# YonghaoHe/LFD-A-Light-and-Fast-Detector

Measured on NVIDIA H100. Metric: images/sec WIDERFACE-S inference 1280x720 batch=8 per GPU bf16, higher is better.
Workload: dtype bf16

## Files before the change

### lfd-a-light-and-fast-detector_b200/build.py

```python
import os
import subprocess
import sys

HERE = os.path.dirname(os.path.abspath(__file__))
CSRC = os.path.join(HERE, 'csrc')
OUT = os.environ.get('LFD_B200_OUT') or os.path.join(HERE, 'liblfd_b200.so')
SOURCES = ['api.cu', 'conv_umma.cu', 'conv_simt.cu', 'postprocess.cu', 'losses.cu', 'train.cu', 'wgrad_umma.cu', 'input.cu']
HEADERS = ['ptx.cuh', 'conv_common.cuh', 'kernels.cuh', 'train.cuh', os.path.join('..', '..', 'include', 'lfd_b200.h')]
NVCC = os.environ.get('NVCC', '/usr/local/cuda/bin/nvcc')
ARCH = ['-gencode', 'arch=compute_90a,code=sm_90a']
FLAGS = ARCH + ['-O3', '-lineinfo', '-std=c++17', '-Xcompiler', '-fPIC',
                '--expt-relaxed-constexpr'] + (['-DLFD_B200_TRACE'] if os.environ.get('LFD_B200_TRACE') else []) + \
        (['-DLFD_B200_TIMELINE'] if os.environ.get('LFD_B200_TIMELINE') else []) + os.environ.get('LFD_B200_EXTRA_FLAGS', '').split()


def _stale():
    if not os.path.exists(OUT):
        return True
    t = os.path.getmtime(OUT)
    deps = [os.path.join(CSRC, s) for s in SOURCES + HEADERS] + [os.path.abspath(__file__)]
    return any(os.path.getmtime(d) > t for d in deps)


_STACK_GUARDED = ('conv_umma_kernel', 'conv_umma_c48_kernel', 'stem4_kernel', 'soft_nms_kernel')
_WGMMA_GUARDED = ('conv_umma_kernel', 'conv_umma_c48_kernel', 'stem4_kernel')
_PTXAS_VERBOSE = ('conv_umma.cu', 'postprocess.cu')


def _check_stack_frames(ptxas_log, limit=64):
    import re
    name = None
    for line in ptxas_log.splitlines():
        m = re.search(r'Function properties for (\S+)', line)
        if m:
            name = m.group(1)
        m = re.search(r'(\d+) bytes stack frame', line)
        if m and name and any(k in name for k in _STACK_GUARDED) and int(m.group(1)) > limit:
            raise RuntimeError('%s has a %s-byte stack frame (limit %d): registers went to local memory' % (name, m.group(1), limit))
        m = re.search(r'\((C75\d\d)\).*wgmma\.mma_async instructions are serialized.*\'(\S+)\'', line)
        if m and any(k in m.group(2) for k in _WGMMA_GUARDED):
            raise RuntimeError('ptxas serialised the wgmma instructions of %s (%s):\n%s' % (m.group(2), m.group(1), line))


def build(force=False, verbose=False):
    if not force and not _stale():
        return OUT
    objs = []
    procs = []
# ... 22 lines not shown
```

### lfd-a-light-and-fast-detector_b200/csrc/conv_common.cuh

```cuda
#pragma once
#include <cuda.h>
#include <cuda_runtime.h>
#include <cuda_bf16.h>
#include <stdint.h>
#include <string.h>
#include "kernels.cuh"

namespace lfd {

enum { MODE_FLAT = 0, MODE_3X3S1 = 1, MODE_3X3S2 = 2, MODE_1X1S2 = 3, MODE_STEM = 4, MODE_STEM4 = 5 };

static constexpr int kMaxStages = 8;
static constexpr int kMaxDevices = 64;
static constexpr int kSmemBarOff = 0;
static constexpr int kSmemTableOff = 512;

struct ConvGeom {
    int N, H, W, Cin, Ho, Wo, Cout, ksize, stride;
    int tail_cout;
    int ds_cout;
    int stem;
    int stem4;
};

// ... 18 lines not shown
    unsigned long long* tl;
    long long* trace;
    int N, H, W, Cin, Ho, Wo, Cout;
    int relu, gn_groups, mode;
    int tiles_x, tiles_per_img, num_tiles;
    unsigned long long magic_tpi, magic_tx;
    int n_px;
    int Cc, stages, b_resident;
    int log2_cpc, log2_cpr;
    uint32_t lbo_a, sbo_a;
    uint32_t a_stage_bytes, b_slice_bytes, stage_bytes, w_total_bytes;
    uint32_t smem_table_off, smem_bias_off, smem_bias2_off, smem_staging_off;
    uint32_t smem_w_off, smem_ring_off;
    int input_format;
    InputTransform xf;
    int f16;
    const __nv_bfloat16* w_s2;
    const float* shift_s2;
    const __nv_bfloat16* w_s3;
    const float* shift_s3;
    int relu_s2, relu_s3, H1, W1;
    int in_words;
    const int* ext;
};

int umma_conv_configure(const ConvGeom& g, int num_sms, UmmaConvParams* out, size_t* smem_bytes, int* grid);
cudaError_t umma_conv_launch(const UmmaConvParams& p, size_t smem, int grid, cudaStream_t st);
int umma_conv_encode_maps(UmmaConvParams* p);

cudaError_t simt_conv_launch(const ConvGeom& g, int Cc, const __nv_bfloat16* in, __nv_bfloat16* out,
                             const __nv_bfloat16* res, const __nv_bfloat16* w, const float* shift,
                             double* stats, int gn_groups, int relu, int f16, cudaStream_t st);

}
```

### lfd-a-light-and-fast-detector_b200/csrc/conv_umma.cu

```cuda
#include <stdlib.h>

#include <type_traits>

#include "conv_common.cuh"
#include "ptx.cuh"

namespace lfd {

static constexpr int kProdThreads = 128;
static constexpr int kConsumerThreads = 256;
static constexpr int kConvThreads = kConsumerThreads + kProdThreads;

#define LFD_LAMBDA_INLINE __attribute__((always_inline))

#ifdef LFD_B200_TRACE
#define LFD_TRACE(role, idx, slot) \
    do { if (p.trace && blockIdx.x == 0 && (idx) < 32) p.trace[((role) * 32 + (idx)) * 4 + (slot)] = clock64(); } while (0)
#define LFD_TRACE_EPI(tr, idx, slot) \
    do { if ((tr) && blockIdx.x == 0 && (idx) < 16) (tr)[(idx) * 8 + (slot)] = clock64(); } while (0)
#else
#define LFD_TRACE(role, idx, slot) ((void)0)
#define LFD_TRACE_EPI(tr, idx, slot) ((void)0)
#endif

// ... 18 lines not shown
    if (MODE == MODE_FLAT) {
        g.tiles_x = 0; g.magic_tx = 0;
        g.tiles_per_img = (g.Ho * p.Wo + 127) / 128;
    } else {
        g.tiles_x = (g.Wo + 7) / 8;
        g.magic_tx = ((1ull << 40) + (uint64_t)g.tiles_x - 1) / (uint64_t)g.tiles_x;
        g.tiles_per_img = g.tiles_x * ((g.Ho + 15) / 16);
    }
    g.num_tiles = g.tiles_per_img * p.N;
    g.magic_tpi = ((1ull << 40) + (uint64_t)g.tiles_per_img - 1) / (uint64_t)g.tiles_per_img;
    return g;
}

struct PxEntry {
    uint32_t src_off;
    uint32_t dst_off;
};
struct PxDelta { int8_t dy, dx; };

static constexpr int kStemRows = 33, kStemCols = 18, kStemPix = kStemRows * kStemCols;
static constexpr int kStemRowBytes = kStemCols * 8;
static constexpr int kStemPerThread = (kStemPix + kProdThreads - 1) / kProdThreads;
static constexpr int kStemPatchBytes = ((kStemRows * kStemRowBytes + 127) / 128) * 128;

LFD_DEVINL float selp_f32(bool c, float a, float b) {
    float r;
    asm("{\n\t.reg .pred p;\n\tsetp.ne.u32 p, %3, 0;\n\tselp.f32 %0, %1, %2, p;\n\t}" : "=f"(r) : "f"(a), "f"(b), "r"((uint32_t)c));
    return r;
}

template <int NV, int N>
LFD_DEVINL void butterfly_step(float* val, int lane) {
    if constexpr (N > 1) {
        constexpr int off = 16 * N / NV;
        const bool upper = (lane & off) != 0;
#pragma unroll
        for (int i = 0; i < N / 2; ++i) {
            const float lo = val[i], hi = val[i + N / 2];
            const float send = selp_f32(upper, lo, hi);
            const float keep = selp_f32(upper, hi, lo);
            val[i] = keep + __shfl_xor_sync(0xffffffffu, send, off);
        }
        butterfly_step<NV, N / 2>(val, lane);
    }
}

// ... 27 lines not shown
    return 0;
}

LFD_DEVINL void wg_bar_sync(int wg) { asm volatile("bar.sync %0, 128;" ::"r"(1 + wg) : "memory"); }

template <int N, int K, bool F16>
LFD_DEVINL void tail_mma(float* acc2, const uint32_t* a2, uint64_t b2desc0) {
#pragma unroll
    for (int kk = 0; kk < K / 16; ++kk) wgmma_rs<N, F16>(acc2, a2 + 4 * kk, b2desc0 + (uint32_t)((kk * 2 * N * 16) >> 4), kk != 0);
}

struct EpiCtx {
    uint32_t stg;
    uint32_t stg_bytes;
    int nbuf;
    int r0, tq;
    int wtid;
    int wg, lane;
#ifdef LFD_B200_TRACE
    long long* tr;
#endif
};

template <int MODE, int NCMAX, bool F16>
LFD_DEVINL void store_tile(const EpiCtx& e, const float* acc, int nc, const float* bias, bool relu, bool res, double* stats,
                           const CUtensorMap* tmap, const CUtensorMap* tmres, int c0, int c1, int n, bool v0, bool v1,
                           uint64_t* res_bar, uint32_t& store_count, uint32_t& res_count) {
    const uint32_t buf = e.stg + (e.nbuf == 2 ? (store_count & 1) * e.stg_bytes : 0u);
#ifdef LFD_B200_TRACE
    const uint32_t tidx = store_count;
#endif
    ++store_count;
    const int row_bytes = nc >= 64 ? 128 : nc * 2;
    const int n_panels = nc >= 64 ? nc / 64 : 1;
    if (e.wtid == 0) {
        LFD_TRACE_EPI(e.tr, tidx, 0);
        if (e.nbuf == 2) bulk_wait_read<1>(); else bulk_wait_read<0>();
        LFD_TRACE_EPI(e.tr, tidx, 1);
        if (res) {
            mbar_arrive_expect_tx(res_bar, 64u * nc * 2u);
            for (int pn = 0; pn < n_panels; ++pn) {
                if (MODE == MODE_FLAT) tma_load_3d(buf + pn * 8192, tmres, pn * 64, c0, n, res_bar);
                else tma_load_4d(buf + pn * 8192, tmres, pn * 64, c0, c1, n, res_bar);
            }
        }
    }
    constexpr int JB = NCMAX / 8 < 8 ? NCMAX / 8 : 4;
    float2 bv[JB];
    auto load_shifts = [&](int j0) LFD_LAMBDA_INLINE {
#pragma unroll
        for (int i = 0; i < JB; ++i)
            if (j0 + i < nc / 8) bv[i] = *reinterpret_cast<const float2*>(bias + 8 * (j0 + i) + 2 * e.tq);
    };
    load_shifts(0);
    wg_bar_sync(e.wg);
    if (res) { mbar_wait(res_bar, res_count & 1); ++res_count; }
    float st[NCMAX == 128 ? 32 : 1];
    const bool stat = NCMAX == 128 && stats != nullptr;
#pragma unroll
    for (int j = 0; j < NCMAX / 8; ++j) {
        if (j < nc / 8) {
            if (j > 0 && j % JB == 0) load_shifts(j);
            const float b0 = bv[j % JB].x, b1 = bv[j % JB].y;
            float s1 = 0.f, s2 = 0.f;
#pragma unroll
            for (int h = 0; h < 2; ++h) {
                const int row = e.r0 + 8 * h;
                const uint32_t swz = NCMAX == 48 ? 0u : (row_bytes == 128 ? (row & 7) : (row_bytes == 64 ? ((row >> 1) & 3) : ((row >> 2) & 1)));
                const uint32_t addr = buf + (uint32_t)(j >> 3) * 8192u + (uint32_t)(row * row_bytes) + ((((uint32_t)j & 7u) ^ swz) << 4) + 4u * e.tq;
                float x0 = acc[4 * j + 2 * h] + b0, x1 = acc[4 * j + 2 * h + 1] + b1;
                if (res) {
                    uint32_t rv;
                    asm volatile("ld.shared.b32 %0, [%1];" : "=r"(rv) : "r"(addr) : "memory");
                    x0 += up_lo<F16>(rv); x1 += up_hi<F16>(rv);
                }
                const uint32_t o = relu ? pack2_relu<F16>(x0, x1) : pack2<F16>(x0, x1);
                asm volatile("st.shared.b32 [%0], %1;" ::"r"(addr), "r"(o) : "memory");
                if (stat && (h ? v1 : v0)) {
                    const float f0 = up_lo<F16>(o), f1 = up_hi<F16>(o);
                    s1 += f0 + f1;
                    s2 = fmaf(f0, f0, fmaf(f1, f1, s2));
                }
            }
            if (NCMAX == 128) { st[j] = s1; st[16 + j] = s2; }
        }
    }
    fence_proxy_async_smem();
    wg_bar_sync(e.wg);
    if (e.wtid == 0) {
        for (int pn = 0; pn < n_panels; ++pn) {
            if (MODE == MODE_FLAT) tma_store_3d(tmap, buf + pn * 8192, pn * 64, c0, n);
            else tma_store_4d(tmap, buf + pn * 8192, pn * 64, c0, c1, n);
        }
        bulk_commit();
        LFD_TRACE_EPI(e.tr, tidx, 2);
    }
    if (NCMAX == 128 && stat) stats_flush<128>(st, e.lane, stats);
}

template <int MODE, int COUT, bool F16, bool EXT, bool DS>
LFD_DEVINL void conv_umma_body(const UmmaConvParams& p) {
    static_assert(!DS || MODE == MODE_3X3S2, "the fused shortcut belongs to a 3x3/s2 conv");
    constexpr int kProd = kProdThreads;
    constexpr int kThreads = kConvThreads;
    constexpr int TAPS = (MODE == MODE_3X3S1 || MODE == MODE_3X3S2) ? 9 : (MODE == MODE_STEM ? 3 : 1);
    extern __shared__ __align__(1024) uint8_t smem[];
    uint64_t* full = reinterpret_cast<uint64_t*>(smem + kSmemBarOff);
    uint64_t* empty = full + kMaxStages;
    uint64_t* wbar = empty + kMaxStages;
    uint64_t* res_bar = wbar + 1;
    PxEntry* table = reinterpret_cast<PxEntry*>(smem + p.smem_table_off);
    PxDelta* delta = reinterpret_cast<PxDelta*>(smem + p.smem_table_off + (size_t)p.n_px * sizeof(PxEntry));
    float* bias = reinterpret_cast<float*>(smem + p.smem_bias_off);
    float* bias2 = reinterpret_cast<float*>(smem + p.smem_bias2_off);
    uint8_t* staging = smem + p.smem_staging_off;
    uint8_t* wres = smem + p.smem_w_off;
    uint8_t* ring = smem + p.smem_ring_off;

    pdl_launch_dependents();
    LFD_TL_BEGIN(p.tl);
    const int tid = threadIdx.x;
    const int warp = tid >> 5;
    const int lane = tid & 31;
    const int SA = p.stages;
    const int cpc = p.Cc >> 3;
// ... 68 lines not shown
        e.tq = lane & 3;
        e.wtid = tid & 127;
        e.wg = wg;
        e.lane = lane;
#ifdef LFD_B200_TRACE
        e.tr = p.trace && e.wtid == 0 ? p.trace + (3 * 32 + wg) * 4 : nullptr;
#endif
        if (e.wtid == 0 && (e.stg & 1023u)) __trap();

        const uint32_t lbo_b = COUT * 16;
        const uint64_t adesc0 = wgmma_desc(0, p.lbo_a, p.sbo_a);
        const uint64_t bdesc0 = wgmma_desc(0, lbo_b, 128);
        const uint32_t a_k16 = (2 * p.lbo_a) >> 4;
        const uint32_t b_k16 = (2 * lbo_b) >> 4;
        const uint32_t b_tap = (cpc * lbo_b) >> 4;
        const uint32_t a_wg = (8u * p.sbo_a * wg) >> 4;
        const int nk16 = p.Cc >> 4;
        const uint64_t b2desc0 = wgmma_desc(smem_u32(smem + p.smem_w2_off), cn2 * 16, 128);
        const int flat_valid = lg.Ho * p.Wo;

        float acc[COUT / 2];
        float acc3[DS ? COUT / 2 : 1];
        uint32_t it = 0, store_count = 0, res_count = 0;
        for (int tile = blockIdx.x, lt = 0; tile < lg.num_tiles; tile += gridDim.x, ++lt) {
            for (int cc = 0; cc < n_cc; ++cc, ++it) {
                const uint32_t s = it % SA, ph = (it / SA) & 1;
                if (cc == 0 && e.wtid == 0) LFD_TRACE(1 + wg, lt, 0);
                mbar_wait(&full[s], ph);
                if (e.wtid == 0) LFD_TRACE(1 + wg, lt, 1);
                fence_proxy_async_smem();
                const uint32_t a_base = smem_u32(ring) + s * p.stage_bytes;
                const uint32_t b_base = p.b_resident ? smem_u32(wres) + cc * p.b_slice_bytes : a_base + p.a_stage_bytes;
                const uint64_t ad = adesc0 + ((a_base >> 4) + a_wg), bd = bdesc0 + (b_base >> 4);
                wgmma_fence_regs<COUT / 2>(acc);
                wgmma_fence();
                for (int k16 = 0; k16 < nk16; ++k16) {
                    const uint64_t adk = ad + (uint32_t)(k16 * a_k16), bdk = bd + (uint32_t)(k16 * b_k16);
#pragma unroll
                    for (int tap = 0; tap < TAPS; ++tap)
                        wgmma_ss<COUT, F16>(acc, adk + (uint32_t)tap_view<MODE>(tap), bdk + (uint32_t)(tap * b_tap), (cc | k16 | tap) != 0);
                }
                if constexpr (DS) {
                    wgmma_fence_regs<COUT / 2>(acc3);
                    for (int k16 = 0; k16 < nk16; ++k16)
                        wgmma_ss<COUT, F16>(acc3, ad + (uint32_t)(k16 * a_k16) + (uint32_t)tap_view<MODE>(4),
                                            b2desc0 + (uint32_t)(((cc * cpc + 2 * k16) * COUT * 16) >> 4), (cc | k16) != 0);
// ... 170 lines not shown
                const int ty = fast_div(t, lg.magic_tx);
                int oy0 = ty * 16, ox0 = (t - ty * lg.tiles_x) * 8;
                iy0 = (MODE == MODE_3X3S1) ? oy0 : 2 * oy0;
                ix0 = (MODE == MODE_3X3S1) ? ox0 : 2 * ox0;
            }
            const __nv_bfloat16* img = p.in + (size_t)n * HW * p.Cin + ch * 8;
            constexpr int kDyMin = (MODE == MODE_1X1S2) ? 0 : -1, kDxMin = kDyMin;
            constexpr int kDyMax = (MODE == MODE_3X3S1) ? 16 : ((MODE == MODE_3X3S2) ? 31 : 30);
            constexpr int kDxMax = (MODE == MODE_3X3S1) ? 8 : ((MODE == MODE_3X3S2) ? 15 : 14);
            const bool interior = MODE == MODE_FLAT ? (ix0 + 128 <= HW)
                                                    : (iy0 + kDyMin >= 0 && ix0 + kDxMin >= 0 && iy0 + kDyMax < lg.H && ix0 + kDxMax < lg.W);
            const __nv_bfloat16* org = img + (ptrdiff_t)(MODE == MODE_FLAT ? ix0 : (iy0 + kDyMin) * p.W + ix0 + kDxMin) * p.Cin;
            for (int cc = 0; cc < n_cc; ++cc, ++it) {
                const uint32_t s = it % SA, ph = (it / SA) & 1;
                if (ptid == 0) LFD_TRACE(0, it, 0);
                mbar_wait(&empty[s], ph ^ 1);
                if (ptid == 0) LFD_TRACE(0, it, 1);
                const uint32_t a_base = smem_u32(ring) + s * p.stage_bytes;
                if (!p.b_resident && ptid == 0) {
                    mbar_arrive_expect_tx(&full[s], p.b_slice_bytes);
                    bulk_g2s(a_base + p.a_stage_bytes, reinterpret_cast<const uint8_t*>(p.w) + (size_t)cc * p.b_slice_bytes,
                             p.b_slice_bytes, &full[s]);
                }
                const __nv_bfloat16* src_cc = img + cc * p.Cc;
                const uint32_t dst_cc = a_base + ch_dst;
                if (MODE == MODE_FLAT) {
                    if (interior) {
                        const __nv_bfloat16* src = org + cc * p.Cc + (size_t)px0 * p.Cin;
                        const size_t sstep = (size_t)pstep * p.Cin;
                        uint32_t dst = dst_cc + px0 * 16;
#pragma unroll 4
                        for (int pxi = px0; pxi < 128; pxi += pstep, src += sstep, dst += pstep * 16) cp_async16_full(dst, src);
                    } else {
#pragma unroll 4
                        for (int pxi = px0; pxi < 128; pxi += pstep) {
                            const int q = ix0 + pxi;
                            const bool ok = q < HW;
                            cp_async16(dst_cc + pxi * 16, src_cc + (ok ? q : 0) * p.Cin, ok);
                        }
                    }
                } else if (interior) {
                    const uint8_t* src = reinterpret_cast<const uint8_t*>(org + cc * p.Cc);
                    const PxEntry* tp = table + px0;
#pragma unroll 4
                    for (int k = 0; k < my_cnt; ++k, tp += pstep) {
                        const uint2 pe = *reinterpret_cast<const uint2*>(tp);
// ... 7 lines not shown
                        const bool ok = ((unsigned)y < (unsigned)lg.H) && ((unsigned)x < (unsigned)lg.W);
                        cp_async16(dst_cc + table[pxi].dst_off, src_cc + (ok ? (y * p.W + x) : 0) * p.Cin, ok);
                    }
                }
                cp_async_mbar_arrive(&full[s]);
                if (ptid == 0) LFD_TRACE(0, it, 2);
            }
        }
        cp_async_wait_all();
        }
    }
    LFD_TL_END(p.tl);
}

template <int MODE, int COUT, bool F16, bool EXT, bool DS>
__global__ void __launch_bounds__(kConvThreads, 1) conv_umma_kernel(const __grid_constant__ UmmaConvParams p) {
    static_assert(COUT != 48, "48-channel outputs run in conv_umma_c48_kernel");
    conv_umma_body<MODE, COUT, F16, EXT, DS>(p);
}

template <int MODE, bool F16, bool EXT, bool DS>
__global__ void __launch_bounds__(kConvThreads, 1) conv_umma_c48_kernel(const __grid_constant__ UmmaConvParams p) {
    conv_umma_body<MODE, 48, F16, EXT, DS>(p);
}

static constexpr int kS4Rows = 67, kS4Cols = 36, kS4Pix = kS4Rows * kS4Cols;
static constexpr int kS4RowBytes = kS4Cols * 8;
static constexpr int kS4PatchBytes = kS4Pix * 8;
static constexpr int kS4PerThread = (kS4Pix + kProdThreads - 1) / kProdThreads;
static constexpr int kS4Batch = 5;
static constexpr int kS4Groups = kS4Rows * 10;
static constexpr int kS4GroupsPerThread = (kS4Groups + kProdThreads - 1) / kProdThreads;
static constexpr int kS4GroupBatch = 3;
static constexpr int kS4PatchOverrun = 768;
LFD_DEVINL constexpr int s4_slot(int a, int b) {
    return ((a & 1) ? ((b & 1) ? 0 : 147) : ((b & 1) ? 291 : 446)) + (a >> 1) * 9 + (b >> 1);
}
static constexpr int kS4Lbo = 599 * 16;
static constexpr int kS4Bar = 0;
static constexpr int kS4Shift = 256;
static constexpr int kS4Staging = 2048;
static constexpr int kS4W0 = kS4Staging + 2 * 8192;
static constexpr int kS4W1 = kS4W0 + 6144;
static constexpr int kS4W2 = kS4W1 + 8192;
static constexpr int kS4W3 = kS4W2 + 73728;
static constexpr int kS4Planes = kS4W3 + 8192;
// ... 324 lines not shown
#pragma unroll
                    for (int j = 0; j < kS4Batch; ++j) {
                        const int q = ptid + (j0 + j) * kProdThreads;
                        if (q >= kS4Pix) break;
                        float f[3];
#pragma unroll
                        for (int k = 0; k < 3; ++k) {
                            f[k] = u8 ? p.xf.apply(k, raw[j][k]) : __uint_as_float(raw[j][k]);
                            if (!ok[j]) f[k] = 0.f;
                        }
                        const uint32_t lo = pack2<F16>(sw ? f[2] : f[0], f[1]), hi = pack2<F16>(sw ? f[0] : f[2], 0.f);
                        asm volatile("st.shared.v2.b32 [%0], {%1, %2};" ::"r"(dst0 + q * 8), "r"(lo), "r"(hi) : "memory");
                    }
                }
            }
            fence_proxy_async_smem();
            mbar_arrive(&full[s]);
            if (ptid == 0) LFD_TRACE(0, lt, 2);
        }
    }
    LFD_TL_END(p.tl);
}

static int configure_with(const ConvGeom& g, int num_sms, int nbuf, UmmaConvParams* out, size_t* smem_bytes, int* grid) {
    UmmaConvParams p;
    memset(&p, 0, sizeof(p));
    p.stg_nbuf = nbuf;
    int mode;
    if (g.stem) {
        if (g.ksize != 3 || g.stride != 2 || g.Cin != 16) return -1;
        mode = MODE_STEM;
    } else if (g.ksize == 1 && g.stride == 1) mode = MODE_FLAT;
    else if (g.ksize == 3 && g.stride == 1) mode = MODE_3X3S1;
    else if (g.ksize == 3 && g.stride == 2) mode = MODE_3X3S2;
    else if (g.ksize == 1 && g.stride == 2) mode = MODE_1X1S2;
    else return -1;
    if (g.Cin % 16 || (g.Cout != 16 && g.Cout != 32 && g.Cout != 48 && g.Cout != 64 && g.Cout != 128)) return -1;
    if ((mode == MODE_3X3S1 || mode == MODE_3X3S2) && g.Cout < 32) return -1;
    p.mode = mode;
    p.N = g.N; p.H = g.H; p.W = g.W; p.Cin = g.Cin; p.Ho = g.Ho; p.Wo = g.Wo; p.Cout = g.Cout;
    const int taps = g.stem ? 3 : g.ksize * g.ksize;
    int px_slots;
    if (mode == MODE_FLAT) {
        p.tiles_x = 0; p.tiles_per_img = (g.Ho * g.Wo + 127) / 128;
        p.n_px = 128; px_slots = 128; p.sbo_a = 128;
    } else {
        p.tiles_x = (g.Wo + 7) / 8;
        p.tiles_per_img = p.tiles_x * ((g.Ho + 15) / 16);
        if (mode == MODE_3X3S1) { p.n_px = 180; px_slots = 180; p.sbo_a = 160; }
        else if (mode == MODE_3X3S2) { p.n_px = 561; px_slots = 594; p.sbo_a = 144; }
        else { p.n_px = 128; px_slots = 128; p.sbo_a = 128; }
    }
    const int plane_slots = px_slots | 1;
    p.lbo_a = plane_slots * 16;
    if (mode == MODE_STEM) { p.lbo_a = 16; p.sbo_a = 2 * kStemRowBytes; }
    p.num_tiles = p.tiles_per_img * g.N;
    if (p.num_tiles >= (1 << 24) || p.tiles_per_img >= (1 << 16)) return -5;
    p.magic_tpi = ((1ull << 40) + p.tiles_per_img - 1) / p.tiles_per_img;
    p.magic_tx = p.tiles_x ? ((1ull << 40) + p.tiles_x - 1) / p.tiles_x : 0;
    const int Cf = g.tail_cout > 0 ? g.tail_cout : g.Cout;
    if (g.ds_cout && (mode != MODE_3X3S2 || g.tail_cout || g.ds_cout != g.Cout)) return -6;
    if (g.tail_cout && (g.tail_cout % 16 || g.tail_cout > 128 || g.tail_cout < 16)) return -4;
    if (g.tail_cout && (g.tail_cout == 48) != (g.Cout == 48)) return -4;
    const size_t staging = (size_t)nbuf * 128 * Cf * 2;
    size_t hoff = kSmemTableOff;
    p.smem_table_off = (uint32_t)hoff;
    if (mode != MODE_FLAT && mode != MODE_STEM) hoff += ((size_t)p.n_px * 10 + 127) & ~(size_t)127;
    p.smem_bias_off = (uint32_t)hoff; hoff += ((size_t)g.Cout * 4 + 15) & ~(size_t)15;
    p.smem_bias2_off = (uint32_t)hoff; hoff += ((size_t)(g.tail_cout + g.ds_cout) * 4 + 15) & ~(size_t)15;
    p.smem_staging_off = (uint32_t)((hoff + 1023) & ~(size_t)1023);
    const size_t fixed = p.smem_staging_off + staging;
    const size_t w2_bytes = g.tail_cout ? ((size_t)g.Cout * g.tail_cout * 2 + 127) & ~(size_t)127
                                        : (g.ds_cout ? ((size_t)g.Cin * g.ds_cout * 2 + 127) & ~(size_t)127 : 0);
    const size_t post = w2_bytes;
    const size_t budget = 224 * 1024 - post;
    const size_t w_total = (size_t)taps * g.Cin * g.Cout * 2;
// ... 114 lines not shown
    const cuuint32_t inner = p.Cf < 64 ? p.Cf : 64;
    const CUtensorMapSwizzle swz = inner * 2 >= 128 ? CU_TENSOR_MAP_SWIZZLE_128B
                                 : (inner * 2 == 96 ? CU_TENSOR_MAP_SWIZZLE_NONE
                                                    : (inner * 2 == 64 ? CU_TENSOR_MAP_SWIZZLE_64B : CU_TENSOR_MAP_SWIZZLE_32B));
    cuuint64_t dims[4], strides[3];
    cuuint32_t box[4], estr[4] = {1, 1, 1, 1};
    cuuint32_t rank;
    if (p.mode == MODE_FLAT) {
        rank = 3;
        dims[0] = Cf; dims[1] = HoWo; dims[2] = p.N;
        strides[0] = Cf * 2; strides[1] = HoWo * Cf * 2;
        box[0] = inner; box[1] = 64; box[2] = 1;
    } else {
        rank = 4;
        dims[0] = Cf; dims[1] = p.Wo; dims[2] = p.Ho; dims[3] = p.N;
        strides[0] = Cf * 2; strides[1] = (cuuint64_t)p.Wo * Cf * 2; strides[2] = HoWo * Cf * 2;
        box[0] = inner; box[1] = 8; box[2] = 8; box[3] = 1;
    }
    CUresult r = fn(tm, CU_TENSOR_MAP_DATA_TYPE_BFLOAT16, rank, const_cast<void*>(ptr), dims, strides, box, estr, CU_TENSOR_MAP_INTERLEAVE_NONE, swz,
                    CU_TENSOR_MAP_L2_PROMOTION_L2_128B, CU_TENSOR_MAP_FLOAT_OOB_FILL_NONE);
    return r == CUDA_SUCCESS ? 0 : -2;
}

int umma_conv_encode_maps(UmmaConvParams* p) {
    if (encode_one(*p, p->out, &p->tm_out)) return -1;
    if (p->res && encode_one(*p, p->res, &p->tm_res)) return -1;
    if (p->Cout3 && encode_one(*p, p->out3, &p->tm_out3)) return -1;
    return 0;
}

static cudaError_t launch_persistent(void (*kernel)(UmmaConvParams), bool* configured, int max_smem, const UmmaConvParams& p, size_t smem,
                                     int grid, cudaStream_t st) {
    int dev = 0;
    if (cudaGetDevice(&dev) != cudaSuccess || dev < 0 || dev >= kMaxDevices) return cudaErrorInvalidDevice;
    if (!configured[dev]) {
        cudaError_t e = cudaFuncSetAttribute(kernel, cudaFuncAttributeMaxDynamicSharedMemorySize, max_smem);
        if (e != cudaSuccess) return e;
        configured[dev] = true;
    }
    cudaLaunchConfig_t cfg;
    memset(&cfg, 0, sizeof(cfg));
    cfg.gridDim = dim3(grid);
    cfg.blockDim = dim3(kConvThreads);
    cfg.dynamicSmemBytes = smem;
    cfg.stream = st;
    cudaLaunchAttribute attr[1];
    attr[0].id = cudaLaunchAttributeProgrammaticStreamSerialization;
    attr[0].val.programmaticStreamSerializationAllowed = 1;
    cfg.attrs = attr;
    cfg.numAttrs = 1;
// ... 5 lines not shown
    static bool configured[kMaxDevices] = {};
    if constexpr (COUT == 48) return launch_persistent(conv_umma_c48_kernel<MODE, F16, EXT, DS>, configured, 224 * 1024, p, smem, grid, st);
    else return launch_persistent(conv_umma_kernel<MODE, COUT, F16, EXT, DS>, configured, 224 * 1024, p, smem, grid, st);
}

template <int MODE, int COUT, bool F16, bool EXT>
static cudaError_t launch_mode_ds(const UmmaConvParams& p, size_t smem, int grid, cudaStream_t st) {
    if constexpr (MODE == MODE_3X3S2)
        if (p.Cout3) return launch_mode_t<MODE, COUT, F16, EXT, true>(p, smem, grid, st);
    return launch_mode_t<MODE, COUT, F16, EXT, false>(p, smem, grid, st);
}

template <bool F16, bool EXT>
static cudaError_t launch_stem4_t(const UmmaConvParams& p, size_t smem, int grid, cudaStream_t st) {
    static bool configured[kMaxDevices] = {};
    return launch_persistent(stem4_kernel<F16, EXT>, configured, kS4Smem, p, smem, grid, st);
}

template <bool F16>
static cudaError_t launch_stem4(const UmmaConvParams& p, size_t smem, int grid, cudaStream_t st) {
    return p.ext ? launch_stem4_t<F16, true>(p, smem, grid, st) : launch_stem4_t<F16, false>(p, smem, grid, st);
}

template <int MODE, int COUT, bool F16>
static cudaError_t launch_mode_e(const UmmaConvParams& p, size_t smem, int grid, cudaStream_t st) {
    return p.ext ? launch_mode_ds<MODE, COUT, F16, true>(p, smem, grid, st) : launch_mode_ds<MODE, COUT, F16, false>(p, smem, grid, st);
}

template <int MODE, int COUT>
static cudaError_t launch_mode(const UmmaConvParams& p, size_t smem, int grid, cudaStream_t st) {
    return p.f16 ? launch_mode_e<MODE, COUT, true>(p, smem, grid, st) : launch_mode_e<MODE, COUT, false>(p, smem, grid, st);
}

template <int MODE>
static cudaError_t launch_cout(const UmmaConvParams& p, size_t smem, int grid, cudaStream_t st) {
    switch (p.Cout) {
        case 16: if constexpr (MODE != MODE_3X3S1 && MODE != MODE_3X3S2) return launch_mode<MODE, 16>(p, smem, grid, st); break;
        case 32: return launch_mode<MODE, 32>(p, smem, grid, st);
        case 48: return launch_mode<MODE, 48>(p, smem, grid, st);
        case 64: return launch_mode<MODE, 64>(p, smem, grid, st);
        case 128: if constexpr (MODE != MODE_STEM) return launch_mode<MODE, 128>(p, smem, grid, st); break;
    }
    return cudaErrorInvalidValue;
}

cudaError_t umma_conv_launch(const UmmaConvParams& p, size_t smem, int grid, cudaStream_t st) {
    switch (p.mode) {
        case MODE_FLAT: return launch_cout<MODE_FLAT>(p, smem, grid, st);
// ... 11 lines not shown
```

### lfd-a-light-and-fast-detector_b200/csrc/ptx.cuh

```cuda
#pragma once
#include <cuda_runtime.h>
#include <cuda_bf16.h>
#include <cuda_fp16.h>
#include <stdint.h>

namespace lfd {

#define LFD_DEVINL __device__ __forceinline__

#ifndef LFD_SPIN_LIMIT
#define LFD_SPIN_LIMIT (1u << 27)
#endif

LFD_DEVINL uint32_t smem_u32(const void* p) { return (uint32_t)__cvta_generic_to_shared(p); }

LFD_DEVINL void mbar_init(uint64_t* bar, uint32_t count) {
    asm volatile("mbarrier.init.shared::cta.b64 [%0], %1;" ::"r"(smem_u32(bar)), "r"(count));
}
LFD_DEVINL void fence_mbar_init() { asm volatile("fence.mbarrier_init.release.cluster;" ::: "memory"); }
LFD_DEVINL void mbar_arrive(uint64_t* bar) {
    asm volatile("mbarrier.arrive.shared::cta.b64 _, [%0];" ::"r"(smem_u32(bar)) : "memory");
}
LFD_DEVINL void mbar_arrive_expect_tx(uint64_t* bar, uint32_t bytes) {
    asm volatile("mbarrier.arrive.expect_tx.shared::cta.b64 _, [%0], %1;" ::"r"(smem_u32(bar)), "r"(bytes) : "memory");
// ... 57 lines not shown
    return pred != 0;
}

LFD_DEVINL void tma_store_3d(const void* tmap, uint32_t src_smem, int c0, int c1, int c2) {
    asm volatile("cp.async.bulk.tensor.3d.global.shared::cta.bulk_group [%0, {%1, %2, %3}], [%4];" ::"l"(tmap), "r"(c0), "r"(c1),
                 "r"(c2), "r"(src_smem)
                 : "memory");
}
LFD_DEVINL void tma_store_4d(const void* tmap, uint32_t src_smem, int c0, int c1, int c2, int c3) {
    asm volatile("cp.async.bulk.tensor.4d.global.shared::cta.bulk_group [%0, {%1, %2, %3, %4}], [%5];" ::"l"(tmap), "r"(c0),
                 "r"(c1), "r"(c2), "r"(c3), "r"(src_smem)
                 : "memory");
}
LFD_DEVINL void tma_load_3d(uint32_t dst_smem, const void* tmap, int c0, int c1, int c2, uint64_t* bar) {
    asm volatile("cp.async.bulk.tensor.3d.shared::cluster.global.mbarrier::complete_tx::bytes [%0], [%1, {%2, %3, %4}], [%5];" ::"r"(dst_smem),
                 "l"(tmap), "r"(c0), "r"(c1), "r"(c2), "r"(smem_u32(bar))
                 : "memory");
}
LFD_DEVINL void tma_load_4d(uint32_t dst_smem, const void* tmap, int c0, int c1, int c2, int c3, uint64_t* bar) {
    asm volatile("cp.async.bulk.tensor.4d.shared::cluster.global.mbarrier::complete_tx::bytes [%0], [%1, {%2, %3, %4, %5}], [%6];" ::"r"(dst_smem),
                 "l"(tmap), "r"(c0), "r"(c1), "r"(c2), "r"(c3), "r"(smem_u32(bar))
                 : "memory");
}
LFD_DEVINL void bulk_commit() { asm volatile("cp.async.bulk.commit_group;" ::: "memory"); }
LFD_DEVINL void bulk_wait_all() { asm volatile("cp.async.bulk.wait_group 0;" ::: "memory"); }
template <int N>
LFD_DEVINL void bulk_wait_read() { asm volatile("cp.async.bulk.wait_group.read %0;" ::"n"(N) : "memory"); }

LFD_DEVINL uint64_t wgmma_desc(uint32_t smem_addr, uint32_t lbo_bytes, uint32_t sbo_bytes) {
    uint64_t d = 0;
    d |= (uint64_t)((smem_addr >> 4) & 0x3FFF);
    d |= (uint64_t)((lbo_bytes >> 4) & 0x3FFF) << 16;
    d |= (uint64_t)((sbo_bytes >> 4) & 0x3FFF) << 32;
    return d;
}
LFD_DEVINL void wgmma_fence() { asm volatile("wgmma.fence.sync.aligned;" ::: "memory"); }
LFD_DEVINL void wgmma_commit() { asm volatile("wgmma.commit_group.sync.aligned;" ::: "memory"); }
template <int N>
LFD_DEVINL void wgmma_wait() { asm volatile("wgmma.wait_group.sync.aligned %0;" ::"n"(N) : "memory"); }
template <int N>
LFD_DEVINL void wgmma_fence_regs(float* d) {
#pragma unroll
    for (int i = 0; i < N; ++i) asm volatile("" : "+f"(d[i])::"memory");
}

template <int N> struct Wgmma;
template <> struct Wgmma<16> {
    template <int TA, int TB>
    static LFD_DEVINL void ss_bf16(float* d, uint64_t a, uint64_t b, uint32_t acc) {
        asm volatile("{\n\t.reg .pred p;\n\tsetp.ne.b32 p, %10, 0;\n\t"
// ... 226 lines not shown
```

Baseline: 11050.

## Add pipelined 3x3/s1 64-channel conv kernel with TMA input loads and double accumulators

Adds a specialised persistent kernel for 3x3 stride-1 64->64 convolutions. Consumers keep two accumulator sets so the wgmma for the next tile is issued before the epilogue of the current one, overlapping tensor-core work with staging, residual prefetch and TMA stores. The producer loads the input halo with a 5D TMA tensor map instead of per-thread copies, which needs a padded plane layout (184 slots). This raises register pressure (two 32-float accumulators) and adds a separate launch path that is chosen only when the eligibility conditions hold.

```diff
diff --git a/lfd-a-light-and-fast-detector_b200/build.py b/lfd-a-light-and-fast-detector_b200/build.py
--- a/lfd-a-light-and-fast-detector_b200/build.py
+++ b/lfd-a-light-and-fast-detector_b200/build.py
@@ -22,8 +22,8 @@
     return any(os.path.getmtime(d) > t for d in deps)
 
 
-_STACK_GUARDED = ('conv_umma_kernel', 'conv_umma_c48_kernel', 'stem4_kernel', 'soft_nms_kernel')
-_WGMMA_GUARDED = ('conv_umma_kernel', 'conv_umma_c48_kernel', 'stem4_kernel')
+_STACK_GUARDED = ('conv_umma_kernel', 'conv_umma_c48_kernel', 'conv_umma_pipe_kernel', 'stem4_kernel', 'soft_nms_kernel')
+_WGMMA_GUARDED = ('conv_umma_kernel', 'conv_umma_c48_kernel', 'conv_umma_pipe_kernel', 'stem4_kernel')
 _PTXAS_VERBOSE = ('conv_umma.cu', 'postprocess.cu')
 
 
diff --git a/lfd-a-light-and-fast-detector_b200/csrc/conv_common.cuh b/lfd-a-light-and-fast-detector_b200/csrc/conv_common.cuh
--- a/lfd-a-light-and-fast-detector_b200/csrc/conv_common.cuh
+++ b/lfd-a-light-and-fast-detector_b200/csrc/conv_common.cuh
@@ -64,6 +64,7 @@
     int relu_s2, relu_s3, H1, W1;
     int in_words;
     const int* ext;
+    CUtensorMap tm_in;
 };
 
 int umma_conv_configure(const ConvGeom& g, int num_sms, UmmaConvParams* out, size_t* smem_bytes, int* grid);
diff --git a/lfd-a-light-and-fast-detector_b200/csrc/conv_umma.cu b/lfd-a-light-and-fast-detector_b200/csrc/conv_umma.cu
--- a/lfd-a-light-and-fast-detector_b200/csrc/conv_umma.cu
+++ b/lfd-a-light-and-fast-detector_b200/csrc/conv_umma.cu
@@ -64,6 +64,8 @@
 static constexpr int kStemRowBytes = kStemCols * 8;
 static constexpr int kStemPerThread = (kStemPix + kProdThreads - 1) / kProdThreads;
 static constexpr int kStemPatchBytes = ((kStemRows * kStemRowBytes + 127) / 128) * 128;
+static constexpr int kS1Pixels = 180;
+static constexpr int kS1PipeSlots = 184;
 
 LFD_DEVINL float selp_f32(bool c, float a, float b) {
     float r;
@@ -137,6 +139,52 @@
 #endif
 };
 
+template <int NCMAX, bool F16>
+LFD_DEVINL void stage_rows(const EpiCtx& e, const float* acc, int nc, const float* bias, bool relu, bool res, bool stat, uint32_t buf,
+                           bool v0, bool v1, uint64_t* res_bar, uint32_t& res_count, float* st) {
+    const int row_bytes = nc >= 64 ? 128 : nc * 2;
+    constexpr int JB = NCMAX / 8 < 8 ? NCMAX / 8 : 4;
+    float2 bv[JB];
+    auto load_shifts = [&](int j0) LFD_LAMBDA_INLINE {
+#pragma unroll
+        for (int i = 0; i < JB; ++i)
+            if (j0 + i < nc / 8) bv[i] = *reinterpret_cast<const float2*>(bias + 8 * (j0 + i) + 2 * e.tq);
+    };
+    load_shifts(0);
+    wg_bar_sync(e.wg);
+    if (res) { mbar_wait(res_bar, res_count & 1); ++res_count; }
+#pragma unroll
+    for (int j = 0; j < NCMAX / 8; ++j) {
+        if (j < nc / 8) {
+            if (j > 0 && j % JB == 0) load_shifts(j);
+            const float b0 = bv[j % JB].x, b1 = bv[j % JB].y;
+            float s1 = 0.f, s2 = 0.f;
+#pragma unroll
+            for (int h = 0; h < 2; ++h) {
+                const int row = e.r0 + 8 * h;
+                const uint32_t swz = NCMAX == 48 ? 0u : (row_bytes == 128 ? (row & 7) : (row_bytes == 64 ? ((row >> 1) & 3) : ((row >> 2) & 1)));
+                const uint32_t addr = buf + (uint32_t)(j >> 3) * 8192u + (uint32_t)(row * row_bytes) + ((((uint32_t)j & 7u) ^ swz) << 4) + 4u * e.tq;
+                float x0 = acc[4 * j + 2 * h] + b0, x1 = acc[4 * j + 2 * h + 1] + b1;
+                if (res) {
+                    uint32_t rv;
+                    asm volatile("ld.shared.b32 %0, [%1];" : "=r"(rv) : "r"(addr) : "memory");
+                    x0 += up_lo<F16>(rv); x1 += up_hi<F16>(rv);
+                }
+                const uint32_t o = relu ? pack2_relu<F16>(x0, x1) : pack2<F16>(x0, x1);
+                asm volatile("st.shared.b32 [%0], %1;" ::"r"(addr), "r"(o) : "memory");
+                if (stat && (h ? v1 : v0)) {
+                    const float f0 = up_lo<F16>(o), f1 = up_hi<F16>(o);
+                    s1 += f0 + f1;
+                    s2 = fmaf(f0, f0, fmaf(f1, f1, s2));
+                }
+            }
+            if (NCMAX == 128) { st[j] = s1; st[16 + j] = s2; }
+        }
+    }
+    fence_proxy_async_smem();
+    wg_bar_sync(e.wg);
+}
+
 template <int MODE, int NCMAX, bool F16>
 LFD_DEVINL void store_tile(const EpiCtx& e, const float* acc, int nc, const float* bias, bool relu, bool res, double* stats,
                            const CUtensorMap* tmap, const CUtensorMap* tmres, int c0, int c1, int n, bool v0, bool v1,
@@ -146,7 +194,6 @@
     const uint32_t tidx = store_count;
 #endif
     ++store_count;
-    const int row_bytes = nc >= 64 ? 128 : nc * 2;
     const int n_panels = nc >= 64 ? nc / 64 : 1;
     if (e.wtid == 0) {
         LFD_TRACE_EPI(e.tr, tidx, 0);
@@ -160,48 +207,9 @@
             }
         }
     }
-    constexpr int JB = NCMAX / 8 < 8 ? NCMAX / 8 : 4;
-    float2 bv[JB];
-    auto load_shifts = [&](int j0) LFD_LAMBDA_INLINE {
-#pragma unroll
-        for (int i = 0; i < JB; ++i)
-            if (j0 + i < nc / 8) bv[i] = *reinterpret_cast<const float2*>(bias + 8 * (j0 + i) + 2 * e.tq);
-    };
-    load_shifts(0);
-    wg_bar_sync(e.wg);
-    if (res) { mbar_wait(res_bar, res_count & 1); ++res_count; }
     float st[NCMAX == 128 ? 32 : 1];
     const bool stat = NCMAX == 128 && stats != nullptr;
-#pragma unroll
-    for (int j = 0; j < NCMAX / 8; ++j) {
-        if (j < nc / 8) {
-            if (j > 0 && j % JB == 0) load_shifts(j);
-            const float b0 = bv[j % JB].x, b1 = bv[j % JB].y;
-            float s1 = 0.f, s2 = 0.f;
-#pragma unroll
-            for (int h = 0; h < 2; ++h) {
-                const int row = e.r0 + 8 * h;
-                const uint32_t swz = NCMAX == 48 ? 0u : (row_bytes == 128 ? (row & 7) : (row_bytes == 64 ? ((row >> 1) & 3) : ((row >> 2) & 1)));
-                const uint32_t addr = buf + (uint32_t)(j >> 3) * 8192u + (uint32_t)(row * row_bytes) + ((((uint32_t)j & 7u) ^ swz) << 4) + 4u * e.tq;
-                float x0 = acc[4 * j + 2 * h] + b0, x1 = acc[4 * j + 2 * h + 1] + b1;
-                if (res) {
-                    uint32_t rv;
-                    asm volatile("ld.shared.b32 %0, [%1];" : "=r"(rv) : "r"(addr) : "memory");
-                    x0 += up_lo<F16>(rv); x1 += up_hi<F16>(rv);
-                }
-                const uint32_t o = relu ? pack2_relu<F16>(x0, x1) : pack2<F16>(x0, x1);
-                asm volatile("st.shared.b32 [%0], %1;" ::"r"(addr), "r"(o) : "memory");
-                if (stat && (h ? v1 : v0)) {
-                    const float f0 = up_lo<F16>(o), f1 = up_hi<F16>(o);
-                    s1 += f0 + f1;
-                    s2 = fmaf(f0, f0, fmaf(f1, f1, s2));
-                }
-            }
-            if (NCMAX == 128) { st[j] = s1; st[16 + j] = s2; }
-        }
-    }
-    fence_proxy_async_smem();
-    wg_bar_sync(e.wg);
+    stage_rows<NCMAX, F16>(e, acc, nc, bias, relu, res, stat, buf, v0, v1, res_bar, res_count, st);
     if (e.wtid == 0) {
         for (int pn = 0; pn < n_panels; ++pn) {
             if (MODE == MODE_FLAT) tma_store_3d(tmap, buf + pn * 8192, pn * 64, c0, n);
@@ -213,9 +221,10 @@
     if (NCMAX == 128 && stat) stats_flush<128>(st, e.lane, stats);
 }
 
-template <int MODE, int COUT, bool F16, bool EXT, bool DS>
+template <int MODE, int COUT, bool F16, bool EXT, bool DS, bool PIPE = false>
 LFD_DEVINL void conv_umma_body(const UmmaConvParams& p) {
     static_assert(!DS || MODE == MODE_3X3S2, "the fused shortcut belongs to a 3x3/s2 conv");
+    static_assert(!PIPE || (MODE == MODE_3X3S1 && COUT == 64 && !DS), "the pipelined consumers run the 3x3/s1 64-channel convs");
     constexpr int kProd = kProdThreads;
     constexpr int kThreads = kConvThreads;
     constexpr int TAPS = (MODE == MODE_3X3S1 || MODE == MODE_3X3S2) ? 9 : (MODE == MODE_STEM ? 3 : 1);
@@ -330,6 +339,93 @@
         float acc[COUT / 2];
         float acc3[DS ? COUT / 2 : 1];
         uint32_t it = 0, store_count = 0, res_count = 0;
+        if constexpr (PIPE) {
+            float accb[COUT / 2];
+            const int T = (int)blockIdx.x < lg.num_tiles ? (lg.num_tiles - 1 - (int)blockIdx.x) / (int)gridDim.x + 1 : 0;
+            const bool has_res = p.res != nullptr;
+            const bool lead = e.wtid == 0;
+#ifdef LFD_B200_TRACE
+#define LFD_PIPE_STAMP(lt, slot) \
+    clock_stamp_if(p.trace + ((1 + wg) * 32 + (lt)) * 4 + (slot), p.trace != nullptr && blockIdx.x == 0 && lead && (lt) < 32)
+#define LFD_PIPE_STAMP_EPI(lt, slot) \
+    clock_stamp_if(p.trace + (3 * 32 + wg) * 4 + (lt) * 8 + (slot), p.trace != nullptr && blockIdx.x == 0 && lead && (lt) < 16)
+#else
+#define LFD_PIPE_STAMP(lt, slot) ((void)0)
+#define LFD_PIPE_STAMP_EPI(lt, slot) ((void)0)
+#endif
+            auto coords = [&](int lt, int& c0, int& c1, int& n) LFD_LAMBDA_INLINE {
+                const int tile = (int)blockIdx.x + lt * (int)gridDim.x;
+                n = fast_div(tile, lg.magic_tpi);
+                const int t = tile - n * lg.tiles_per_img;
+                const int ty = fast_div(t, lg.magic_tx);
+                c1 = ty * 16 + wg * 8; c0 = (t - ty * lg.tiles_x) * 8;
+            };
+            auto fetch_res = [&](int lt, bool pred) LFD_LAMBDA_INLINE {
+                int c0, c1, n;
+                coords(lt, c0, c1, n);
+                tma_load_4d_expect_if(e.stg + (uint32_t)(lt & 1) * e.stg_bytes, &p.tm_res, 0, c0, c1, n, &res_bar[wg], 64u * COUT * 2u,
+                                      pred && lead && has_res);
+            };
+            constexpr uint32_t kAk16 = 2 * kS1PipeSlots, kBk16 = 2 * COUT, kBtap = 8 * COUT;
+            auto issue = [&](float* a, int lt) LFD_LAMBDA_INLINE {
+                const uint32_t s = (uint32_t)lt % SA, ph = ((uint32_t)lt / SA) & 1;
+                LFD_PIPE_STAMP(lt, 0);
+                mbar_wait(&full[s], ph);
+                LFD_PIPE_STAMP(lt, 1);
+                fence_proxy_async_smem();
+                const uint64_t ad = adesc0 + (((smem_u32(ring) + s * p.stage_bytes) >> 4) + a_wg), bd = bdesc0 + (smem_u32(wres) >> 4);
+                wgmma_fence_regs<COUT / 2>(a);
+                wgmma_fence();
+#pragma unroll
+                for (int k16 = 0; k16 < 4; ++k16)
+#pragma unroll
+                    for (int tap = 0; tap < 9; ++tap)
+                        wgmma_ss<COUT, F16>(a, ad + (uint32_t)(k16 * kAk16) + (uint32_t)tap_view<MODE>(tap),
+                                            bd + (uint32_t)(k16 * kBk16) + (uint32_t)(tap * kBtap), (k16 | tap) != 0);
+            };
+            auto epilogue = [&](float* cur, int lt) LFD_LAMBDA_INLINE {
+                wgmma_fence_regs<COUT / 2>(cur);
+                LFD_PIPE_STAMP(lt, 2);
+                __syncwarp();
+                mbar_arrive_if(&empty[(uint32_t)lt % SA], lane == 0);
+                LFD_PIPE_STAMP_EPI(lt, 0);
+                int c0, c1, n;
+                coords(lt, c0, c1, n);
+                const uint32_t buf = e.stg + (uint32_t)(lt & 1) * e.stg_bytes;
+                LFD_PIPE_STAMP_EPI(lt, 1);
+                stage_rows<COUT, F16>(e, cur, COUT, bias, (bool)p.relu, has_res, false, buf, false, false, &res_bar[wg], res_count, nullptr);
+                tma_store_4d_commit_if(&p.tm_out, buf, 0, c0, c1, n, lead);
+                LFD_PIPE_STAMP_EPI(lt, 2);
+                bulk_wait_read_if<1>(lead);
+                fetch_res(lt + 1, lt + 1 < T);
+            };
+            auto step = [&](float* cur, float* nxt, int lt) LFD_LAMBDA_INLINE {
+                issue(nxt, lt + 1);
+                wgmma_commit();
+                wgmma_wait<1>();
+                epilogue(cur, lt);
+            };
+            if (T > 0) {
+                fetch_res(0, true);
+                issue(acc, 0);
+                wgmma_commit();
+                int lt = 0;
+                for (; lt + 2 < T; lt += 2) {
+                    step(acc, accb, lt);
+                    step(accb, acc, lt + 1);
+                }
+                if (lt + 1 < T) {
+                    step(acc, accb, lt);
+                    wgmma_wait<0>();
+                    epilogue(accb, lt + 1);
+                } else {
+                    wgmma_wait<0>();
+                    epilogue(acc, lt);
+                }
+            }
+#undef LFD_PIPE_STAMP
+#undef LFD_PIPE_STAMP_EPI
+        } else
         for (int tile = blockIdx.x, lt = 0; tile < lg.num_tiles; tile += gridDim.x, ++lt) {
             for (int cc = 0; cc < n_cc; ++cc, ++it) {
                 const uint32_t s = it % SA, ph = (it / SA) & 1;
@@ -546,6 +642,20 @@
                     bulk_g2s(a_base + p.a_stage_bytes, reinterpret_cast<const uint8_t*>(p.w) + (size_t)cc * p.b_slice_bytes,
                              p.b_slice_bytes, &full[s]);
                 }
+                if constexpr (PIPE) {
+                    if (!EXT || interior) {
+                        if (ptid == 0) {
+                            mbar_arrive_expect_tx(&full[s], (uint32_t)kS1Pixels * 64u * 2u);
+#pragma unroll
+                            for (int c = 0; c < 8; ++c)
+                                tma_load_5d(a_base + (uint32_t)c * p.lbo_a, &p.tm_in, 0, c, ix0 - 1, iy0 - 1, n, &full[s]);
+                        } else {
+                            mbar_arrive(&full[s]);
+                        }
+                        if (ptid == 0) LFD_TRACE(0, it, 2);
+                        continue;
+                    }
+                }
                 const __nv_bfloat16* src_cc = img + cc * p.Cc;
                 const uint32_t dst_cc = a_base + ch_dst;
                 if (MODE == MODE_FLAT) {
@@ -599,6 +709,11 @@
 template <int MODE, bool F16, bool EXT, bool DS>
 __global__ void __launch_bounds__(kConvThreads, 1) conv_umma_c48_kernel(const __grid_constant__ UmmaConvParams p) {
     conv_umma_body<MODE, 48, F16, EXT, DS>(p);
+}
+
+template <bool F16, bool EXT>
+__global__ void __launch_bounds__(kConvThreads, 1) conv_umma_pipe_kernel(const __grid_constant__ UmmaConvParams p) {
+    conv_umma_body<MODE_3X3S1, 64, F16, EXT, false, true>(p);
 }
 
 static constexpr int kS4Rows = 67, kS4Cols = 36, kS4Pix = kS4Rows * kS4Cols;
@@ -969,6 +1084,10 @@
     LFD_TL_END(p.tl);
 }
 
+static bool pipe_geom(const ConvGeom& g) {
+    return !g.stem && !g.stem4 && g.ksize == 3 && g.stride == 1 && g.Cin == 64 && g.Cout == 64 && !g.tail_cout && !g.ds_cout;
+}
+
 static int configure_with(const ConvGeom& g, int num_sms, int nbuf, UmmaConvParams* out, size_t* smem_bytes, int* grid) {
     UmmaConvParams p;
     memset(&p, 0, sizeof(p));
@@ -994,11 +1113,11 @@
     } else {
         p.tiles_x = (g.Wo + 7) / 8;
         p.tiles_per_img = p.tiles_x * ((g.Ho + 15) / 16);
-        if (mode == MODE_3X3S1) { p.n_px = 180; px_slots = 180; p.sbo_a = 160; }
+        if (mode == MODE_3X3S1) { p.n_px = kS1Pixels; px_slots = kS1Pixels; p.sbo_a = 160; }
         else if (mode == MODE_3X3S2) { p.n_px = 561; px_slots = 594; p.sbo_a = 144; }
         else { p.n_px = 128; px_slots = 128; p.sbo_a = 128; }
     }
-    const int plane_slots = px_slots | 1;
+    const int plane_slots = pipe_geom(g) ? kS1PipeSlots : px_slots | 1;
     p.lbo_a = plane_slots * 16;
     if (mode == MODE_STEM) { p.lbo_a = 16; p.sbo_a = 2 * kStemRowBytes; }
     p.num_tiles = p.tiles_per_img * g.N;
@@ -1159,10 +1278,23 @@
     return r == CUDA_SUCCESS ? 0 : -2;
 }
 
+static int encode_input(const UmmaConvParams& p, CUtensorMap* tm) {
+    EncodeTiledFn fn = encode_fn();
+    if (!fn) return -1;
+    const cuuint64_t C = p.Cin;
+    cuuint64_t dims[5] = {8, C / 8, (cuuint64_t)p.W, (cuuint64_t)p.H, (cuuint64_t)p.N};
+    cuuint64_t strides[4] = {16, C * 2, (cuuint64_t)p.W * C * 2, (cuuint64_t)p.H * p.W * C * 2};
+    cuuint32_t box[5] = {8, 1, 10, 18, 1}, estr[5] = {1, 1, 1, 1, 1};
+    CUresult r = fn(tm, CU_TENSOR_MAP_DATA_TYPE_BFLOAT16, 5, const_cast<__nv_bfloat16*>(p.in), dims, strides, box, estr,
+                    CU_TENSOR_MAP_INTERLEAVE_NONE, CU_TENSOR_MAP_SWIZZLE_NONE, CU_TENSOR_MAP_L2_PROMOTION_L2_128B, CU_TENSOR_MAP_FLOAT_OOB_FILL_NONE);
+    return r == CUDA_SUCCESS ? 0 : -2;
+}
+
 int umma_conv_encode_maps(UmmaConvParams* p) {
     if (encode_one(*p, p->out, &p->tm_out)) return -1;
     if (p->res && encode_one(*p, p->res, &p->tm_res)) return -1;
     if (p->Cout3 && encode_one(*p, p->out3, &p->tm_out3)) return -1;
+    if (p->mode == MODE_3X3S1 && p->lbo_a == kS1PipeSlots * 16 && encode_input(*p, &p->tm_in)) return -1;
     return 0;
 }
 
@@ -1214,8 +1346,20 @@
     return p.ext ? launch_stem4_t<F16, true>(p, smem, grid, st) : launch_stem4_t<F16, false>(p, smem, grid, st);
 }
 
+template <bool F16, bool EXT>
+static cudaError_t launch_pipe_t(const UmmaConvParams& p, size_t smem, int grid, cudaStream_t st) {
+    static bool configured[kMaxDevices] = {};
+    return launch_persistent(conv_umma_pipe_kernel<F16, EXT>, configured, 224 * 1024, p, smem, grid, st);
+}
+
+static bool pipe_eligible(const UmmaConvParams& p) {
+    return p.Cin == 64 && p.Cc == 64 && p.lbo_a == kS1PipeSlots * 16 && p.b_resident && p.stg_nbuf == 2 && !p.Cout2 && !p.stats;
+}
+
 template <int MODE, int COUT, bool F16>
 static cudaError_t launch_mode_e(const UmmaConvParams& p, size_t smem, int grid, cudaStream_t st) {
+    if constexpr (MODE == MODE_3X3S1 && COUT == 64)
+        if (pipe_eligible(p)) return p.ext ? launch_pipe_t<F16, true>(p, smem, grid, st) : launch_pipe_t<F16, false>(p, smem, grid, st);
     return p.ext ? launch_mode_ds<MODE, COUT, F16, true>(p, smem, grid, st) : launch_mode_ds<MODE, COUT, F16, false>(p, smem, grid, st);
 }
 
diff --git a/lfd-a-light-and-fast-detector_b200/csrc/ptx.cuh b/lfd-a-light-and-fast-detector_b200/csrc/ptx.cuh
--- a/lfd-a-light-and-fast-detector_b200/csrc/ptx.cuh
+++ b/lfd-a-light-and-fast-detector_b200/csrc/ptx.cuh
@@ -103,10 +103,43 @@
                  "l"(tmap), "r"(c0), "r"(c1), "r"(c2), "r"(c3), "r"(smem_u32(bar))
                  : "memory");
 }
+LFD_DEVINL void tma_load_5d(uint32_t dst_smem, const void* tmap, int c0, int c1, int c2, int c3, int c4, uint64_t* bar) {
+    asm volatile("cp.async.bulk.tensor.5d.shared::cluster.global.mbarrier::complete_tx::bytes [%0], [%1, {%2, %3, %4, %5, %6}], [%7];"
+                 ::"r"(dst_smem), "l"(tmap), "r"(c0), "r"(c1), "r"(c2), "r"(c3), "r"(c4), "r"(smem_u32(bar))
+                 : "memory");
+}
 LFD_DEVINL void bulk_commit() { asm volatile("cp.async.bulk.commit_group;" ::: "memory"); }
 LFD_DEVINL void bulk_wait_all() { asm volatile("cp.async.bulk.wait_group 0;" ::: "memory"); }
 template <int N>
 LFD_DEVINL void bulk_wait_read() { asm volatile("cp.async.bulk.wait_group.read %0;" ::"n"(N) : "memory"); }
+
+LFD_DEVINL void mbar_arrive_if(uint64_t* bar, bool pred) {
+    asm volatile("{\n\t.reg .pred p;\n\tsetp.ne.u32 p, %1, 0;\n\t@p mbarrier.arrive.shared::cta.b64 _, [%0];\n\t}"
+                 ::"r"(smem_u32(bar)), "r"((uint32_t)pred) : "memory");
+}
+LFD_DEVINL void tma_store_4d_commit_if(const void* tmap, uint32_t src_smem, int c0, int c1, int c2, int c3, bool pred) {
+    asm volatile("{\n\t.reg .pred p;\n\tsetp.ne.u32 p, %6, 0;\n\t"
+                 "@p cp.async.bulk.tensor.4d.global.shared::cta.bulk_group [%0, {%1, %2, %3, %4}], [%5];\n\t"
+                 "@p cp.async.bulk.commit_group;\n\t}"
+                 ::"l"(tmap), "r"(c0), "r"(c1), "r"(c2), "r"(c3), "r"(src_smem), "r"((uint32_t)pred) : "memory");
+}
+template <int N>
+LFD_DEVINL void bulk_wait_read_if(bool pred) {
+    asm volatile("{\n\t.reg .pred p;\n\tsetp.ne.u32 p, %1, 0;\n\t@p cp.async.bulk.wait_group.read %0;\n\t}"
+                 ::"n"(N), "r"((uint32_t)pred) : "memory");
+}
+LFD_DEVINL void tma_load_4d_expect_if(uint32_t dst_smem, const void* tmap, int c0, int c1, int c2, int c3, uint64_t* bar, uint32_t bytes,
+                                      bool pred) {
+    asm volatile("{\n\t.reg .pred p;\n\tsetp.ne.u32 p, %8, 0;\n\t"
+                 "@p mbarrier.arrive.expect_tx.shared::cta.b64 _, [%6], %7;\n\t"
+                 "@p cp.async.bulk.tensor.4d.shared::cluster.global.mbarrier::complete_tx::bytes [%0], [%1, {%2, %3, %4, %5}], [%6];\n\t}"
+                 ::"r"(dst_smem), "l"(tmap), "r"(c0), "r"(c1), "r"(c2), "r"(c3), "r"(smem_u32(bar)), "r"(bytes), "r"((uint32_t)pred)
+                 : "memory");
+}
+LFD_DEVINL void clock_stamp_if(long long* dst, bool pred) {
+    asm volatile("{\n\t.reg .pred p;\n\t.reg .u64 t;\n\tsetp.ne.u32 p, %1, 0;\n\tmov.u64 t, %%clock64;\n\t@p st.global.u64 [%0], t;\n\t}"
+                 ::"l"(dst), "r"((uint32_t)pred) : "memory");
+}
 
 LFD_DEVINL uint64_t wgmma_desc(uint32_t smem_addr, uint32_t lbo_bytes, uint32_t sbo_bytes) {
     uint64_t d = 0;
```

Measured after the change: 11510 (median of 6 runs). 1.04x the previous value.
